# ohinder/OnePhase.jl

Measured on AMD Instinct MI355X. Metric: KKT factor+solve/sec (fp64) at n+m~1e5, nnz~2e6, higher is better.
Workload: dtype f64

## Files before the change

onephase.jl_amd/csrc/solve.hip:

```cpp
#include "numeric.h"
#include "solve_sparse.h"

#include <algorithm>
#include <cstdio>
#include <cstdlib>

namespace okkt {

#define OKKT_HIP_TRY(expr)                                                         \
  do {                                                                             \
    hipError_t e__ = (expr);                                                       \
    if (e__ != hipSuccess)                                                         \
      return std::string(#expr) + ": " + hipGetErrorString(e__);                   \
  } while (0)

typedef double d4_t __attribute__((ext_vector_type(4)));
typedef double d2_t __attribute__((ext_vector_type(2)));

constexpr int kSB = kSolveBlock;
#ifndef OKKT_SOLVE_SPLITS
#define OKKT_SOLVE_SPLITS 8
#endif
constexpr int kCS = OKKT_SOLVE_SPLITS;
static_assert(kSB / kCS >= 128 && (kCS & (kCS - 1)) == 0, "the block-product kernels need column splits of at least 128 columns (64 gave wrong results: found in round 3)");
// ... 482 lines not shown
  }
  const int kq = min(CW, pend - q0);
  const double* X = P.xinv + P.xinv_pos[s] + off + (size_t)q0 * ld;
  const int ic = min(i, kb - 1);
  const int64_t gcb = P.bigcol_base[s];
  if (ver && b > 0) flow_wait(ver, (c0 + q0) >> 5, ((c0 + q0 + kq - 1) >> 5) - ((c0 + q0) >> 5) + 1, vwant, nullptr, 0ull, P.counters + 5);
  for (int c = tid; c < CW; c += 256) {
    double w[R];
#pragma unroll
    for (int r = 0; r < R; ++r) w[r] = 0.0;
    if (c < kq) {
      if (b == 0) fwd_gather<R>(P, gcb, col0, k, q0 + c, w);
      else {
#pragma unroll
        for (int r = 0; r < R; ++r) w[r] = ver ? ld_agent(&P.xwork[(size_t)r * P.xw_stride + col0 + c0 + q0 + c]) : P.xwork[(size_t)r * P.xw_stride + col0 + c0 + q0 + c];
      }
    }
#pragma unroll
    for (int r = 0; r < R; ++r) wj[r][c] = w[r];
  }
  __syncthreads();
  double a[R];
#pragma unroll
  for (int r = 0; r < R; ++r) a[r] = 0.0;
  for (int p0 = wv * (CW / 4); p0 < min(kq, (wv + 1) * (CW / 4)); p0 += 32) {
    double v[32];
#pragma unroll
    for (int q = 0; q < 32; ++q) v[q] = X[(size_t)min(p0 + q, kq - 1) * ld + ic];
#pragma unroll
    for (int q = 0; q < 32; ++q) {
      const double vv = p0 + q < kq ? v[q] : 0.0;
#pragma unroll
      for (int r = 0; r < R; ++r) a[r] += vv * wj[r][min(p0 + q, CW - 1)];
    }
  }
#pragma unroll
  for (int r = 0; r < R; ++r) part[wv][r][lane] = a[r];
  __syncthreads();
  if (wv == 0 && i < kb)
#pragma unroll
    for (int r = 0; r < R; ++r) {
      const double v = (part[0][r][lane] + part[1][r][lane]) + (part[2][r][lane] + part[3][r][lane]);
      if (AG) st_agent(&yp[(size_t)r * kCS * kSB + i], v); else yp[(size_t)r * kCS * kSB + i] = v;
    }
  return true;
}
template <int R>
__global__ __launch_bounds__(256) void k_fwd_y(DevPlan P, const int* __restrict__ list, int b) {
  if (P.solve_mid) { const int s = list[blockIdx.y]; if (P.sn_col0[s + 1] - P.sn_col0[s] <= P.solve_mid) return; }
  (void)fwd_y_body<R, false>(P, list[blockIdx.y], b, (int)blockIdx.x, (int)blockIdx.z);
}

constexpr int kUpdRows = 64;
template <int R, int ROWS = kUpdRows>
__device__ __forceinline__ void fwd_upd_body(const DevPlan& P, int s, int b, int bx, double* sm, const unsigned long long* counter, unsigned long long epoch,
                                             unsigned long long* ver = nullptr, unsigned long long vbase = 0, int rb_abs = -1, int first = -1, long long yexp = -1) {
  constexpr int GW = ROWS / 2, NG = 256 / GW;
  double* yj = sm;
  double* part = sm + (size_t)R * kSB;
  const int tid = threadIdx.x, l32 = tid % GW, hw = tid / GW;
  const int col0 = P.sn_col0[s];
  const int k = P.sn_col0[s + 1] - col0;
  const int f = (int)(P.row_ptr[s + 1] - P.row_ptr[s]);
  int c0, kb, ld; int64_t off;
  xblock(k, b, c0, kb, ld, off);
  if (kb <= 0) return;
  const int rbeg = c0 + kb;
  const int rb = rb_abs >= 0 ? rb_abs : rbeg + bx * ROWS;
  const bool is_first = first >= 0 ? first != 0 : bx == 0;
  if (!is_first && rb >= f) return;
  const int vt0 = rb >> 5, vnt = rb < f ? min(ROWS / 32, (f - rb + 31) >> 5) : 0;
  if (ver) flow_wait(ver, vt0, b > 0 ? vnt : 0, vbase + (unsigned long long)b, counter, (epoch << 20) + (unsigned long long)yexp, P.counters + 5);
  else if (counter) front_wait64(counter, epoch, ((kb + 63) / 64) * kCS, P.counters + 5);
  const double* yp = P.ypart + P.ypart_pos[s] + (ver ? (size_t)b * kMaxRhs * kCS * kSB : 0);
  for (int p = tid; p < kSB; p += 256) {
    const int pc = min(p, kb - 1);
#pragma unroll
    for (int r = 0; r < R; ++r) {
      const double y = counter ? sum_splits_agent(yp + (size_t)r * kCS * kSB + pc) : sum_splits(yp + (size_t)r * kCS * kSB + pc);
      yj[r * kSB + p] = p < kb ? y : 0.0;
      if (is_first && p < kb) P.zwork[(size_t)r * P.xw_stride + col0 + c0 + p] = y / P.dvals[col0 + c0 + p];
    }
  }
  __syncthreads();
  if (rb >= f) return;
  const int r0 = rb + 2 * l32;
  const bool pair_ok = f >= 2;
  const int pr = pair_ok ? max(min(r0, f - 2), 0) : 0;
  const double* Lp = P.arena + P.front_pos[s] + (size_t)c0 * f + pr;
  double a0[R], a1[R];
#pragma unroll
  for (int r = 0; r < R; ++r) { a0[r] = 0.0; a1[r] = 0.0; }
  for (int p0 = hw; p0 < kb; p0 += 16 * NG) {
    d2_t v[16];
#pragma unroll
    for (int u = 0; u < 16; ++u) {
      const int p = min(p0 + NG * u, kb - 1);
      if (pair_ok) __builtin_memcpy(&v[u], Lp + (size_t)p * f, 16);
      else { v[u][0] = Lp[(size_t)p * f]; v[u][1] = 0.0; }
    }
#pragma unroll
    for (int u = 0; u < 16; ++u) {
      const int p = p0 + NG * u;
      if (p < kb) {
#pragma unroll
        for (int r = 0; r < R; ++r) { const double y = yj[r * kSB + p]; a0[r] += v[u][0] * y; a1[r] += v[u][1] * y; }
      }
    }
  }
#pragma unroll
  for (int r = 0; r < R; ++r) {
    part[((size_t)hw * R + r) * ROWS + 2 * l32] = a0[r];
    part[((size_t)hw * R + r) * ROWS + 2 * l32 + 1] = a1[r];
  }
  __syncthreads();
  if (tid < ROWS) {
    const int ln = tid >> 1, e = tid & 1;
    const int r0l = rb + 2 * ln;
    const int prl = pair_ok ? max(min(r0l, f - 2), 0) : 0;
    const int sh = r0l - prl;
    const int rowv = pair_ok ? prl + e : prl;
    const bool valid = pair_ok ? (sh == 0 || (sh == 1 && e == 1)) : (e == 0 && r0l < f);
    if (valid && rowv >= rbeg && rowv < f) {
      const int64_t gcb = P.bigcol_base[s];
      double w[R];
      if (b == 0) fwd_gather<R>(P, gcb, col0, k, rowv, w);
      else {
#pragma unroll
        for (int r = 0; r < R; ++r) w[r] = ver ? ld_agent(fwd_slot<R>(P, s, col0, k, rowv, r)) : *fwd_slot<R>(P, s, col0, k, rowv, r);
      }
#pragma unroll
      for (int r = 0; r < R; ++r) {
        double sum = 0.0;
#pragma unroll
        for (int h = 0; h < NG; ++h) sum += part[((size_t)h * R + r) * ROWS + tid];
        if (ver) st_agent(fwd_slot<R>(P, s, col0, k, rowv, r), w[r] - sum); else *fwd_slot<R>(P, s, col0, k, rowv, r) = w[r] - sum;
      }
    }
  }
  if (ver) flow_publish(ver, vt0, vnt, vbase + (unsigned long long)b + 1ull);
}

template <int R, int ROWS = kUpdRows>
__global__ __launch_bounds__(256) void k_fwd_upd(DevPlan P, const int* __restrict__ list, int b) {
  extern __shared__ __attribute__((aligned(16))) double sm[];
  fwd_upd_body<R, ROWS>(P, list[blockIdx.y], b, (int)blockIdx.x, sm, nullptr, 0ull);
}
template <int R>
__global__ __launch_bounds__(256) void k_fwd_wide_fused(DevPlan P, const int* __restrict__ list, int b, int ny, unsigned long long* __restrict__ counters, unsigned long long epoch) {
  extern __shared__ __attribute__((aligned(16))) double sm[];
  const int s = list[blockIdx.y];
  const int x = (int)blockIdx.x;
  if (x < ny * kCS) {
    if (fwd_y_body<R, true>(P, s, b, x % ny, x / ny)) front_arrive64(counters + s, epoch);
  } else {
    fwd_upd_body<R>(P, s, b, x - ny * kCS, sm, counters + s, epoch);
  }
}

constexpr int kFlowBlocks = 96;
constexpr int kFlowNear = 32;
struct SweepFlow {
  int nblk;
  int base[kFlowBlocks + 1];
  short nprod[kFlowBlocks];
};
template <int R>
__global__ __launch_bounds__(256) void k_fwd_wide_flow(DevPlan P, const int* __restrict__ list, SweepFlow T, unsigned long long* __restrict__ counters, unsigned long long epoch) {
  extern __shared__ __attribute__((aligned(16))) double sm[];
  const int s = list[blockIdx.x];
  const int t = (int)blockIdx.y;
  int b = 0;
  while (b + 1 < T.nblk && t >= T.base[b + 1]) ++b;
  const int idx = t - T.base[b];
  const int k = P.sn_col0[s + 1] - P.sn_col0[s];
  int c0, kb, ld; int64_t off;
  xblock(k, b, c0, kb, ld, off);
  if (kb <= 0) return;
  unsigned long long* ver = P.sver + P.sver_pos[s];
  const unsigned long long vbase = epoch << 12;
  const int nprod = T.nprod[b];
  const int f = (int)(P.row_ptr[s + 1] - P.row_ptr[s]);
  unsigned long long* ycnt = ver + ((f + 31) >> 5) + 2 + b;
  if (idx < nprod) {
    const int ny = nprod / kCS;
    if (fwd_y_body<R, true>(P, s, b, idx % ny, idx / ny, ver, vbase + (unsigned long long)b)) front_arrive64(ycnt, epoch);
    return;
  }
  const int j = idx - nprod;
  const int t0 = (c0 + kb) >> 5;
  const long long yexp = (long long)((kb + 63) / 64) * kCS;
  if (j < kFlowNear) fwd_upd_body<R, 32>(P, s, b, j, sm, ycnt, epoch, ver, vbase, 32 * (t0 + j), j == 0, yexp);
  else fwd_upd_body<R, 64>(P, s, b, j, sm, ycnt, epoch, ver, vbase, 32 * (t0 + kFlowNear) + 64 * (j - kFlowNear), 0, yexp);
}

template <int R, bool SC1>
__device__ __forceinline__ void bwd_pre_body(const DevPlan& P, int s, int xblk) {
  const int lane = threadIdx.x & 63, wv = threadIdx.x >> 6;
  const int col0 = P.sn_col0[s];
  const int k = P.sn_col0[s + 1] - col0;
  const int f = (int)(P.row_ptr[s + 1] - P.row_ptr[s]);
  const int c = xblk * 4 + wv;
  if (c >= k || f == k) return;
  const int* rows = P.rows + P.row_ptr[s];
  const double* col = P.arena + P.front_pos[s] + (size_t)c * f;
  double acc[R];
#pragma unroll
  for (int q = 0; q < R; ++q) acc[q] = 0.0;
  int r = k + lane;
  for (; r + 7 * 64 < f; r += 8 * 64) {
    int ri[8];
    double lv[8];
#pragma unroll
    for (int u = 0; u < 8; ++u) { ri[u] = rows[r + 64 * u]; lv[u] = col[r + 64 * u]; }
#pragma unroll
    for (int q = 0; q < R; ++q) {
      double xv[8];
#pragma unroll
      for (int u = 0; u < 8; ++u) xv[u] = P.xwork[(size_t)q * P.xw_stride + ri[u]];
#pragma unroll
      for (int u = 0; u < 8; ++u) acc[q] += lv[u] * xv[u];
    }
  }
  for (; r < f; r += 64) {
    const double l = col[r];
    const int g = rows[r];
#pragma unroll
    for (int q = 0; q < R; ++q) acc[q] += l * P.xwork[(size_t)q * P.xw_stride + g];
  }
#pragma unroll
  for (int q = 0; q < R; ++q) {
    double a = acc[q];
    for (int o = 32; o > 0; o >>= 1) a += __shfl_down(a, o, 64);
    if (lane == 0) {
      double* zp = &P.zwork[(size_t)q * P.xw_stride + col0 + c];
      if (SC1) st_agent(zp, *zp - a); else *zp -= a;
    }
  }
}
template <int R>
__global__ __launch_bounds__(256) void k_bwd_pre(DevPlan P, const int* __restrict__ list) {
  bwd_pre_body<R, false>(P, list[blockIdx.y], (int)blockIdx.x);
}

template <int R>
__device__ __forceinline__ void bwd_thin_body(const DevPlan& P, int s, int NB, int* counter, double (*tk)[128]) {
  const int tid = threadIdx.x;
  const int col0 = P.sn_col0[s];
  const int k = P.sn_col0[s + 1] - col0;
  const double* X = P.invl + P.invl_pos[s];
  const int c = tid >> 1, h = tid & 1;
  const double* xcol = X + (size_t)min(c, NB - 1) * NB;
  double v[64];
#pragma unroll
  for (int q = 0; q < 64; ++q) v[q] = xcol[min(h * 64 + q, NB - 1)];
  if (counter) {
    const int f = (int)(P.row_ptr[s + 1] - P.row_ptr[s]);
    const int expected = f > k ? (k + 3) / 4 : 0;
    front_wait(counter, expected, P.counters + 5);
    if (tid == 0) __hip_atomic_store(counter, 0, __ATOMIC_RELAXED, __HIP_MEMORY_SCOPE_AGENT);
  }
  if (tid < 128)
#pragma unroll
    for (int r = 0; r < R; ++r) {
      const double* zp = &P.zwork[(size_t)r * P.xw_stride + col0 + min(tid, max(k - 1, 0))];
      tk[r][tid] = tid < k ? (counter ? ld_agent(zp) : *zp) : 0.0;
    }
  __syncthreads();
#pragma unroll
  for (int r = 0; r < R; ++r) {
    double a = 0.0;
#pragma unroll
    for (int q = 0; q < 64; ++q) a += (h * 64 + q < NB) ? v[q] * tk[r][h * 64 + q] : 0.0;
    a += __shfl_xor(a, 1, 64);
    if (h == 0 && c < k) P.xwork[(size_t)r * P.xw_stride + col0 + c] = a;
  }
}
template <int R>
__global__ __launch_bounds__(256) void k_bwd_thin(DevPlan P, const int* __restrict__ list, int NB) {
  __shared__ double tk[R][128];
  bwd_thin_body<R>(P, list[blockIdx.x], NB, nullptr, tk);
}
template <int R>
__global__ __launch_bounds__(256) void k_bwd_thin_fused(DevPlan P, const int* __restrict__ list, int NB, int* __restrict__ counters) {
  __shared__ double tk[R][128];
  const int s = list[blockIdx.y];
  if (blockIdx.x + 1 < gridDim.x) {
    const int k = P.sn_col0[s + 1] - P.sn_col0[s];
    const int f = (int)(P.row_ptr[s + 1] - P.row_ptr[s]);
    if ((int)blockIdx.x * 4 >= k || f == k) return;
    bwd_pre_body<R, true>(P, s, (int)blockIdx.x);
    front_signal_add(counters + s);
  } else {
    bwd_thin_body<R>(P, s, NB, counters + s, tk);
  }
}

// ... 2 lines not shown
  constexpr int RW = kSB / kCS;
  __shared__ double zj[R][RW];
  const int tid = threadIdx.x, lane = tid & 63, wv = tid >> 6;
  const int col0 = P.sn_col0[s];
  const int k = P.sn_col0[s + 1] - col0;
  int c0, kb, ld; int64_t off;
  xblock(k, b, c0, kb, ld, off);
  if (kb <= 0) return false;
  if (bx * 64 >= kb) return false;
  double* xp = P.ypart + P.ypart_pos[s] + (size_t)rq * kSB;
  const int i0 = bx * 64 + wv * 16;
  const int q0 = rq * RW;
  if (q0 >= kb || q0 + RW - 1 < bx * 64) {
    if (lane < 16 && i0 + lane < kb)
#pragma unroll
      for (int r = 0; r < R; ++r) { if (AG) st_agent(&xp[(size_t)r * kCS * kSB + i0 + lane], 0.0); else xp[(size_t)r * kCS * kSB + i0 + lane] = 0.0; }
    return true;
  }
  const int kq = min(RW, kb - q0);
  const double* X = P.xinv + P.xinv_pos[s] + off + q0;
  for (int p = tid; p < RW; p += 256)
#pragma unroll
    for (int r = 0; r < R; ++r) zj[r][p] = p < kq ? P.zwork[(size_t)r * P.xw_stride + col0 + c0 + q0 + p] : 0.0;
  __syncthreads();
#pragma unroll 1
  for (int g = 0; g < 16; g += 4) {
    double v[4][RW / 64];
#pragma unroll
    for (int q = 0; q < 4; ++q) {
      const double* xc = X + (size_t)min(i0 + g + q, kb - 1) * ld;
#pragma unroll
      for (int t = 0; t < RW / 64; ++t) v[q][t] = xc[min(lane + 64 * t, kq - 1)];
    }
#pragma unroll
    for (int q = 0; q < 4; ++q) {
#pragma unroll
      for (int r = 0; r < R; ++r) {
        double a = 0.0;
#pragma unroll
        for (int t = 0; t < RW / 64; ++t) a += (lane + 64 * t < kq) ? v[q][t] * zj[r][lane + 64 * t] : 0.0;
        for (int o = 32; o > 0; o >>= 1) a += __shfl_down(a, o, 64);
        if (lane == 0 && i0 + g + q < kb) { if (AG) st_agent(&xp[(size_t)r * kCS * kSB + i0 + g + q], a); else xp[(size_t)r * kCS * kSB + i0 + g + q] = a; }
      }
    }
  }
  return true;
}
template <int R>
__global__ __launch_bounds__(256) void k_bwd_x(DevPlan P, const int* __restrict__ list, int b) {
  if (P.solve_mid) { const int s = list[blockIdx.y]; if (P.sn_col0[s + 1] - P.sn_col0[s] <= P.solve_mid) return; }
  (void)bwd_x_body<R, false>(P, list[blockIdx.y], b, (int)blockIdx.x, (int)blockIdx.z);
}

template <int R, int COLS = 64>
__device__ __forceinline__ void bwd_upd_body(const DevPlan& P, int s, int b, int bx, double* sm, const unsigned long long* counter, unsigned long long epoch) {
  const int tid = threadIdx.x, lane = tid & 63, wv = tid >> 6;
  const int col0 = P.sn_col0[s];
  const int k = P.sn_col0[s + 1] - col0;
  const int f = (int)(P.row_ptr[s + 1] - P.row_ptr[s]);
  int c0, kb, ld; int64_t off;
  xblock(k, b, c0, kb, ld, off);
  if (kb <= 0) return;
  const int nupd = (c0 + COLS - 1) / COLS;
  if (bx > nupd) return;
  if (counter) front_wait64(counter, epoch, ((kb + 63) / 64) * kCS, P.counters + 5);
  const double* xp = P.ypart + P.ypart_pos[s];
  for (int p = tid; p < kSB; p += 256) {
    const int pc = min(p, kb - 1);
#pragma unroll
    for (int r = 0; r < R; ++r) {
      const double x = counter ? sum_splits_agent(xp + (size_t)r * kCS * kSB + pc) : sum_splits(xp + (size_t)r * kCS * kSB + pc);
      sm[r * kSB + p] = p < kb ? x : 0.0;
    }
  }
  __syncthreads();
  if (bx == nupd) {
    for (int p = tid; p < kb; p += 256)
#pragma unroll
      for (int r = 0; r < R; ++r) P.xwork[(size_t)r * P.xw_stride + col0 + c0 + p] = sm[r * kSB + p];
    return;
  }
  const double* Lrow = P.arena + P.front_pos[s] + c0;
#pragma unroll 1
  for (int g = 0; g < COLS / 4; g += 2) {
    const int cb = bx * COLS + wv * (COLS / 4) + g;
    if (cb >= c0) break;
    double acc[2][R];
#pragma unroll
    for (int q = 0; q < 2; ++q)
#pragma unroll
      for (int r = 0; r < R; ++r) acc[q][r] = 0.0;
    for (int t0 = 0; t0 < kb; t0 += 64 * 16) {
      double v[2][16];
#pragma unroll
      for (int q = 0; q < 2; ++q) {
        const double* col = Lrow + (size_t)min(cb + q, c0 - 1) * f;
#pragma unroll
        for (int t = 0; t < 16; ++t) v[q][t] = col[min(t0 + lane + 64 * t, kb - 1)];
      }
#pragma unroll
      for (int t = 0; t < 16; ++t) {
        const int p = t0 + lane + 64 * t;
        if (p < kb) {
#pragma unroll
          for (int r = 0; r < R; ++r) {
            const double x = sm[r * kSB + p];
            acc[0][r] += v[0][t] * x;
            acc[1][r] += v[1][t] * x;
          }
        }
      }
    }
#pragma unroll
    for (int q = 0; q < 2; ++q)
#pragma unroll
      for (int r = 0; r < R; ++r) {
        double a = acc[q][r];
        for (int o = 32; o > 0; o >>= 1) a += __shfl_down(a, o, 64);
        if (lane == 0 && cb + q < c0) P.zwork[(size_t)r * P.xw_stride + col0 + cb + q] -= a;
      }
  }
}
template <int R, int COLS = 64>
__global__ __launch_bounds__(256) void k_bwd_upd(DevPlan P, const int* __restrict__ list, int b) {
  extern __shared__ __attribute__((aligned(16))) double sm[];
  bwd_upd_body<R, COLS>(P, list[blockIdx.y], b, (int)blockIdx.x, sm, nullptr, 0ull);
}
template <int R>
__global__ __launch_bounds__(256) void k_bwd_wide_fused(DevPlan P, const int* __restrict__ list, int b, int nx, unsigned long long* __restrict__ counters, unsigned long long epoch) {
  extern __shared__ __attribute__((aligned(16))) double sm[];
  const int s = list[blockIdx.y];
  const int x = (int)blockIdx.x;
  if (x < nx * kCS) {
    if (bwd_x_body<R, true>(P, s, b, x % nx, x / nx)) front_arrive64(counters + s, epoch);
  } else {
    bwd_upd_body<R>(P, s, b, x - nx * kCS, sm, counters + s, epoch);
  }
}

constexpr int kMidThreads = 1024;
__device__ __forceinline__ void mid_load_x(const double* Xb, int o, int NB, double (&xr)[4]) {
  const int tid = threadIdx.x;
#pragma unroll
  for (int u = 0; u < 4; ++u) {
    const int idx = tid + kMidThreads * u, i = idx & 63, j = idx >> 6;
    xr[u] = Xb[(o + i) + (size_t)(o + j) * NB];
  }
}
__device__ __forceinline__ void mid_store_x(const double (&xr)[4], double* xb) {
  const int tid = threadIdx.x;
#pragma unroll
  for (int u = 0; u < 4; ++u) {
    const int idx = tid + kMidThreads * u, i = idx & 63, j = idx >> 6;
    xb[i + j * 65] = xr[u];
  }
}
template <int R>
__global__ __launch_bounds__(kMidThreads) void k_fwd_mid(DevPlan P, const int* __restrict__ list, int NB) {
  extern __shared__ __attribute__((aligned(16))) double sm[];
  __shared__ double xb[2][64 * 65], ys[R][64];
  double (*part)[R][64] = (double (*)[R][64])(sm + (size_t)R * kSB);
  const int s = list[blockIdx.x];
  const int tid = threadIdx.x;
  const int col0 = P.sn_col0[s];
  const int k = P.sn_col0[s + 1] - col0;
  const int f = (int)(P.row_ptr[s + 1] - P.row_ptr[s]);
  if (k > P.solve_mid) return;
  const double* F = P.arena + P.front_pos[s];
  const double* X = P.invl + P.invl_pos[s];
  const int q = tid & 3, pr = tid >> 2;
  auto load_panel = [&](int c0, int pbase, d2_t (&v)[16]) {
    const int nb = min(64, k - c0);
    const int p = pbase + 2 * pr;
    if (c0 < k && p < k) {
      const bool two = p + 1 < k;
      const double* Lr = F + (size_t)(c0 + 16 * q) * f + (two ? p : p - 1);
#pragma unroll
      for (int u = 0; u < 16; ++u) __builtin_memcpy(&v[u], Lr + (size_t)min(u, max(nb - 1 - 16 * q, 0)) * f, 16);
    }
// ... 316 lines not shown
        ssched.push_back(s);
        L.wide_maxf = std::max(L.wide_maxf, N.sn_f[s]); L.wide_maxk = std::max(L.wide_maxk, N.sn_k[s]); L.wide_mink = std::min(L.wide_mink, N.sn_k[s]);
        if (xinv_pos[s] < 0) {
          const int64_t k = N.sn_k[s];
          const int64_t nfull = k / kSB, last = k - nfull * kSB, lastp = (last + 127) / 128 * 128;
          xinv_pos[s] = xtot;
          xtot += nfull * (int64_t)kSB * kSB + lastp * lastp;
          ypart_pos[s] = ytot;
          ytot += (int64_t)kMaxRhs * kCS * kSB * (N.solve_flow ? (k + kSB - 1) / kSB : 1);
          sver_pos[s] = vtot;
          vtot += (N.sn_f[s] + 31) / 32 + 2 + (k + kSB - 1) / kSB;
        }
      }
    }
  };
  build(N.levels, N.slevels);
  build(N.levels_top, N.slevels_top);
  std::string e;
  if (!(e = up(N, ssched, &d.ssched)).empty()) return e;
  N.ssched_host = ssched;
  if (!(e = up(N, xinv_pos, &d.xinv_pos)).empty()) return e;
  if (!(e = up(N, ypart_pos, &d.ypart_pos)).empty()) return e;
  if (!(e = up(N, ythin_pos, &d.ythin_pos)).empty()) return e;
  if (!(e = dz(N, (size_t)ttot, &d.ythin)).empty()) return e;
  if (!(e = dz(N, (size_t)xtot, &d.xinv)).empty()) return e;
  if (!(e = dz(N, (size_t)xtot, &d.xtmp)).empty()) return e;
  if (!(e = dz(N, (size_t)ytot, &d.ypart)).empty()) return e;
  if (!(e = up(N, sver_pos, &d.sver_pos)).empty()) return e;
  {
    double* rawv = nullptr;
    if (!(e = dz(N, (size_t)vtot + 1, &rawv)).empty()) return e;
    d.sver = (unsigned long long*)rawv;
  }
  {
    double* raw = nullptr;
    if (!(e = dz(N, (size_t)ns + 64, &raw)).empty()) return e;
    N.solve_flags = (int*)raw;
    N.solve_counters = (int*)raw + ns + 16;
    N.solve_epoch = 0;
    double* raw64 = nullptr;
    if (!(e = dz(N, (size_t)ns + 8, &raw64)).empty()) return e;
    N.solve_counters64 = (unsigned long long*)raw64;
    N.solve_epoch64 = 0;
  }
  for (const void* fn : {(const void*)k_fwd_wide_fused<1>, (const void*)k_fwd_wide_fused<2>, (const void*)k_fwd_wide_fused<4>, (const void*)k_bwd_wide_fused<1>,
                         (const void*)k_bwd_wide_fused<2>, (const void*)k_bwd_wide_fused<4>})
    OKKT_HIP_TRY(hipFuncSetAttribute(fn, hipFuncAttributeMaxDynamicSharedMemorySize, 160 * 1024 - 4096 - 16 * 1024));
  for (const void* fn : {(const void*)k_fwd_mid<1>, (const void*)k_fwd_mid<2>, (const void*)k_fwd_mid<4>, (const void*)k_bwd_mid<1>, (const void*)k_bwd_mid<2>, (const void*)k_bwd_mid<4>})
    OKKT_HIP_TRY(hipFuncSetAttribute(fn, hipFuncAttributeMaxDynamicSharedMemorySize, 80 * 1024));
  for (const void* fn : {(const void*)k_fwd_upd<1>, (const void*)k_fwd_upd<2>, (const void*)k_fwd_upd<4>, (const void*)k_bwd_upd<1>,
                         (const void*)k_bwd_upd<2>, (const void*)k_bwd_upd<4>, (const void*)k_fwd_upd<1, 32>, (const void*)k_fwd_upd<2, 32>, (const void*)k_fwd_upd<4, 32>, (const void*)k_bwd_upd<1, 16>, (const void*)k_bwd_upd<2, 16>, (const void*)k_bwd_upd<4, 16>, (const void*)k_fs_small<256, 1>, (const void*)k_fs_small<256, 2>,
                         (const void*)k_fs_small<256, 4>, (const void*)k_bs_small<256, 1>, (const void*)k_bs_small<256, 2>, (const void*)k_bs_small<256, 4>})
    OKKT_HIP_TRY(hipFuncSetAttribute(fn, hipFuncAttributeMaxDynamicSharedMemorySize, 160 * 1024 - 4096));
  return "";
}

std::string solve_invert_enqueue(Numeric& N, hipStream_t st, const SolveLevel& L, int b_lo, int b_hi) {
  if (!L.wide_cnt) return "";
  DevPlan P = N.d;
  const int* list = P.ssched + L.wide_off;
  const int nblk = (L.wide_maxk + kSB - 1) / kSB;
  b_hi = std::min(b_hi, nblk);
  if (b_lo >= b_hi) return "";
  const int nbk = b_hi - b_lo;
  const int maxkb = std::min(kSB, L.wide_maxk - b_lo * kSB);
  const int ldmax = std::min(kSB, (maxkb + 127) / 128 * 128);
  hipLaunchKernelGGL(k_xinv_init, dim3(ldmax / N.nb, 1, (unsigned)(L.wide_cnt * nbk)), dim3(256), 0, st, P, list, b_lo, nbk, N.nb);
  for (int sz = N.nb; sz < ldmax; sz *= 2) {
    const int npair = (ldmax + 2 * sz - 1) / (2 * sz);
    const int tiles = ((sz + 63) / 64) * ((sz + 63) / 64);
    hipLaunchKernelGGL(k_xinv_gemm<0>, dim3(tiles, npair, (unsigned)(L.wide_cnt * nbk)), dim3(256), 0, st, P, list, b_lo, nbk, sz);
    hipLaunchKernelGGL(k_xinv_gemm<1>, dim3(tiles, npair, (unsigned)(L.wide_cnt * nbk)), dim3(256), 0, st, P, list, b_lo, nbk, sz);
  }
  OKKT_HIP_TRY(hipGetLastError());
  return "";
}

struct SweepView {
  const std::vector<LevelSchedule>& levels;
  const std::vector<SolveLevel>& sl;
  const int* sched;
  const int* ssched;
  bool own, waits;
};

template <int R>
static std::string fwd_enqueue_r(Numeric& N, const SweepView& V, hipStream_t st, int l_lo, int l_hi) {
  DevPlan P = N.d;
  const std::vector<LevelSchedule>& levels = V.levels;
  const std::vector<SolveLevel>& sl = V.sl;
  const bool flow = V.own && V.waits && N.flow_levels >= 2 && N.flow_flags && l_lo == 0 && l_hi >= N.flow_levels;
  for (size_t l = (size_t)l_lo; l < std::min((size_t)l_hi, levels.size()); ++l) {
    const LevelSchedule& L = levels[l];
    if (flow && l == 0) {
      const size_t lds = (size_t)R * N.flow_maxf * sizeof(double);
      int* flags = N.flow_flags + (size_t)N.d.nsuper;
      const int ep = ++N.flow_epoch;
      static const int drop = getenv("OKKT_DEBUG_DROP_HANDOFF") ? atoi(getenv("OKKT_DEBUG_DROP_HANDOFF")) : 0;
      const int wep = ep + ((drop & 2) ? (1 << 20) : 0);
      if (N.flow_maxf <= 32) hipLaunchKernelGGL((k_fs_small<64, R, true>), dim3(N.flow_cnt), dim3(64), lds, st, P, P.sched + N.flow_off, N.flow_maxf, flags, ep, wep);
      else hipLaunchKernelGGL((k_fs_small<256, R, true>), dim3(N.flow_cnt), dim3(256), lds, st, P, P.sched + N.flow_off, N.flow_maxf, flags, ep, wep);
      l = (size_t)N.flow_levels - 1;
      continue;
    }
    for (int c = 0; c < 3; ++c) {
      const Segment& g = L.seg[c];
      if (!g.cnt) continue;
      const size_t lds = (size_t)R * g.maxf * sizeof(double);
      if (c == 0) hipLaunchKernelGGL((k_fs_small<64, R>), dim3(g.cnt), dim3(64), lds, st, P, V.sched + g.off, g.maxf, (int*)nullptr, 0, 0);
      else hipLaunchKernelGGL((k_fs_small<256, R>), dim3(g.cnt), dim3(256), lds, st, P, V.sched + g.off, g.maxf, (int*)nullptr, 0, 0);
    }
    if (V.own && (size_t)l < N.inv_level_pending.size() && N.inv_level_pending[l]) {
      OKKT_HIP_TRY(hipStreamWaitEvent(st, N.inv_level_events[l], 0));
      N.inv_level_pending[l] = 0;
    }
    const SolveLevel& S = sl[l];
    if (S.thin_cnt && V.waits && N.solve_fuse && N.solve_flags) {
      hipLaunchKernelGGL(k_fwd_thin_fused<R>, dim3((S.thin_maxr + 127) / 128 + 1, S.thin_cnt), dim3(256), 0, st, P, V.ssched + S.thin_off, N.nb, N.solve_flags, N.solve_epoch);
    } else if (S.thin_cnt) {
      hipLaunchKernelGGL(k_fwd_thin_y<R>, dim3(S.thin_cnt), dim3(256), 0, st, P, V.ssched + S.thin_off, N.nb);
      if (S.thin_maxr > 0) hipLaunchKernelGGL(k_fwd_thin_upd<R>, dim3((S.thin_maxr + 127) / 128, S.thin_cnt), dim3(256), 0, st, P, V.ssched + S.thin_off);
    }
    if (S.wide_cnt) {
      const int* list = V.ssched + S.wide_off;
      const int nblk = (S.wide_maxk + kSB - 1) / kSB;
      const size_t lds = ((size_t)R * kSB + (size_t)8 * R * kUpdRows) * sizeof(double);
      bool flow_done = false;
      if (V.waits && N.solve_flow && N.solve_counters64 && P.sver && nblk <= kFlowBlocks) {
        SweepFlow T;
        T.nblk = nblk;
        int64_t tot = 0;
        for (int b = 0; b < nblk; ++b) {
          const int kbmax = std::min(kSB, S.wide_maxk - b * kSB);
          const int rem = std::max(S.wide_maxf - b * kSB, 0);
          T.base[b] = (int)tot;
          T.nprod[b] = (short)(((kbmax + 63) / 64) * kCS);
          tot += T.nprod[b] + kFlowNear + std::max(0, (rem + 32 - 32 * kFlowNear + 63) / 64);
        }
        T.base[nblk] = (int)tot;
        if (tot <= 65535) {
          hipLaunchKernelGGL(k_fwd_wide_flow<R>, dim3(S.wide_cnt, (unsigned)tot), dim3(256), lds, st, P, list, T, N.solve_counters64, ++N.solve_epoch64);
          flow_done = true;
        }
      }
      for (int b = 0; b < nblk && !flow_done; ++b) {
        const int kbmax = std::min(kSB, S.wide_maxk - b * kSB);
        const int rem = std::max(S.wide_maxf - b * kSB, 0);
        const int ny = (kbmax + 63) / 64, nupd = std::max(1, (rem + kUpdRows - 1) / kUpdRows);
        if (V.waits && N.solve_fuse && N.solve_counters64 && ny * kCS * S.wide_cnt <= N.solve_fuse_wide_max) {
          hipLaunchKernelGGL(k_fwd_wide_fused<R>, dim3(ny * kCS + nupd, S.wide_cnt), dim3(256), lds, st, P, list, b, ny, N.solve_counters64, ++N.solve_epoch64);
        } else {
          if (P.solve_mid && b == 0 && S.wide_mink <= P.solve_mid) hipLaunchKernelGGL(k_fwd_mid<R>, dim3(S.wide_cnt), dim3(kMidThreads), (size_t)R * (kSB + 16 * 64) * sizeof(double), st, P, list, N.nb);
          if (!P.solve_mid || S.wide_maxk > P.solve_mid) hipLaunchKernelGGL(k_fwd_y<R>, dim3(ny, S.wide_cnt, kCS), dim3(256), 0, st, P, list, b);
          if (N.solve_split_small && nupd * S.wide_cnt < N.solve_split_small) hipLaunchKernelGGL((k_fwd_upd<R, 32>), dim3(std::max(1, (rem + 31) / 32), S.wide_cnt), dim3(256), lds, st, P, list, b);
          else hipLaunchKernelGGL(k_fwd_upd<R>, dim3(nupd, S.wide_cnt), dim3(256), lds, st, P, list, b);
        }
      }
    }
  }
  OKKT_HIP_TRY(hipGetLastError());
  return "";
}

template <int R>
static std::string bwd_enqueue_r(Numeric& N, const SweepView& V, hipStream_t st, int l_lo, int l_hi) {
  DevPlan P = N.d;
  const std::vector<LevelSchedule>& levels = V.levels;
  const std::vector<SolveLevel>& sl = V.sl;
  const bool flow = V.own && V.waits && N.flow_levels >= 2 && N.flow_flags && l_lo == 0 && l_hi >= N.flow_levels;
  for (int l = std::min(l_hi, (int)levels.size()) - 1; l >= l_lo; --l) {
    const LevelSchedule& L = levels[l];
    if (flow && l == N.flow_levels - 1) {
      const size_t lds = (size_t)R * N.flow_maxf * sizeof(double);
      int* flags = N.flow_flags + (size_t)2 * N.d.nsuper;
      const int ep = ++N.flow_epoch;
      if (N.flow_maxf <= 32) hipLaunchKernelGGL((k_bs_small<64, R, true>), dim3(N.flow_cnt), dim3(64), lds, st, P, P.sched + N.flow_off, N.flow_maxf, flags, ep);
      else hipLaunchKernelGGL((k_bs_small<256, R, true>), dim3(N.flow_cnt), dim3(256), lds, st, P, P.sched + N.flow_off, N.flow_maxf, flags, ep);
      break;
    }
    const SolveLevel& S = sl[l];
    if (S.wide_cnt) {
      const int* list = V.ssched + S.wide_off;
      if (S.wide_maxf > 0) hipLaunchKernelGGL(k_bwd_pre<R>, dim3((S.wide_maxk + 3) / 4, S.wide_cnt), dim3(256), 0, st, P, list);
      const int nblk = (S.wide_maxk + kSB - 1) / kSB;
      const size_t lds = (size_t)R * kSB * sizeof(double);
      for (int b = nblk - 1; b >= 0; --b) {
        const int kbmax = std::min(kSB, S.wide_maxk - b * kSB);
        const int nx = (kbmax + 63) / 64, nupd = (b * kSB + 63) / 64 + 1;
        if (V.waits && N.solve_fuse && N.solve_counters64 && nx * kCS * S.wide_cnt <= N.solve_fuse_wide_max) {
          hipLaunchKernelGGL(k_bwd_wide_fused<R>, dim3(nx * kCS + nupd, S.wide_cnt), dim3(256), lds, st, P, list, b, nx, N.solve_counters64, ++N.solve_epoch64);
        } else {
          if (P.solve_mid && b == 0 && S.wide_mink <= P.solve_mid) hipLaunchKernelGGL(k_bwd_mid<R>, dim3(S.wide_cnt), dim3(kMidThreads), (size_t)R * (kSB + 16 * 64) * sizeof(double), st, P, list, N.nb);
          if (!P.solve_mid || S.wide_maxk > P.solve_mid) hipLaunchKernelGGL(k_bwd_x<R>, dim3(nx, S.wide_cnt, kCS), dim3(256), 0, st, P, list, b);
          if (P.solve_mid && S.wide_maxk <= P.solve_mid) continue;
          if (N.solve_split_small && nupd * S.wide_cnt < N.solve_split_small) hipLaunchKernelGGL((k_bwd_upd<R, 16>), dim3((b * kSB + 15) / 16 + 1, S.wide_cnt), dim3(256), lds, st, P, list, b);
          else hipLaunchKernelGGL(k_bwd_upd<R>, dim3(nupd, S.wide_cnt), dim3(256), lds, st, P, list, b);
        }
      }
    }
    if (S.thin_cnt && V.waits && N.solve_fuse && N.solve_counters) {
      hipLaunchKernelGGL(k_bwd_thin_fused<R>, dim3((S.thin_maxk + 3) / 4 + 1, S.thin_cnt), dim3(256), 0, st, P, V.ssched + S.thin_off, N.nb, N.solve_counters);
    } else if (S.thin_cnt) {
      const int* list = V.ssched + S.thin_off;
      if (S.thin_maxr > 0) hipLaunchKernelGGL(k_bwd_pre<R>, dim3((S.thin_maxk + 3) / 4, S.thin_cnt), dim3(256), 0, st, P, list);
      hipLaunchKernelGGL(k_bwd_thin<R>, dim3(S.thin_cnt), dim3(256), 0, st, P, list, N.nb);
    }
    for (int c = 0; c < 3; ++c) {
      const Segment& g = L.seg[c];
      if (!g.cnt) continue;
      const size_t lds = (size_t)R * g.maxf * sizeof(double);
      if (c == 0) hipLaunchKernelGGL((k_bs_small<64, R>), dim3(g.cnt), dim3(64), lds, st, P, V.sched + g.off, g.maxf, (int*)nullptr, 0);
      else hipLaunchKernelGGL((k_bs_small<256, R>), dim3(g.cnt), dim3(256), lds, st, P, V.sched + g.off, g.maxf, (int*)nullptr, 0);
    }
  }
  OKKT_HIP_TRY(hipGetLastError());
  return "";
}


static std::string sweep(Numeric& N, bool fwd, const SweepView& V, hipStream_t st, int R, int l_lo = 0, int l_hi = 1 << 30) {
  if (fwd) return R == 1 ? fwd_enqueue_r<1>(N, V, st, l_lo, l_hi) : (R == 2 ? fwd_enqueue_r<2>(N, V, st, l_lo, l_hi) : fwd_enqueue_r<4>(N, V, st, l_lo, l_hi));
  return R == 1 ? bwd_enqueue_r<1>(N, V, st, l_lo, l_hi) : (R == 2 ? bwd_enqueue_r<2>(N, V, st, l_lo, l_hi) : bwd_enqueue_r<4>(N, V, st, l_lo, l_hi));
}

static std::string sweep_which(Numeric& N, bool fwd, int which, int R) {
  if (which != 0) return sweep(N, fwd, SweepView{N.levels_top, N.slevels_top, N.d.sched, N.d.ssched, false, true}, N.stream, R);
  return sweep(N, fwd, SweepView{N.levels, N.slevels, N.d.sched, N.d.ssched, true, true}, N.stream, R);
}

std::string solve_fwd_enqueue(Numeric& N, int which, int R) {
  if (which == 0 && N.inv_wait) { OKKT_HIP_TRY(hipStreamWaitEvent(N.stream, N.inv_event, 0)); N.inv_wait = false; }
  ++N.solve_epoch;
  return sweep_which(N, true, which, R);
}
std::string solve_bwd_enqueue(Numeric& N, int which, int R) {
  return sweep_which(N, false, which, R);
}

std::string solve_fwd_enqueue_lists(Numeric& N, const SweepLists& L, int R) {
  if (N.inv_wait) { OKKT_HIP_TRY(hipStreamWaitEvent(N.stream, N.inv_event, 0)); N.inv_wait = false; }
  ++N.solve_epoch;
  return sweep(N, true, SweepView{*L.levels, *L.slevels, L.sched, L.ssched, true, false}, N.stream, R);
}
std::string solve_bwd_enqueue_lists(Numeric& N, const SweepLists& L, int R) {
  return sweep(N, false, SweepView{*L.levels, *L.slevels, L.sched, L.ssched, true, false}, N.stream, R);
}

std::string schur_gather_enqueue(Numeric& N, double* d_r2, int nr, int R) {
  const int ns = N.sn_k[N.schur_sn], col0 = N.d.n - ns;
// ... 74 lines not shown
```

Measured before the change: 57.90.

## Software-pipeline panel loads in sparse triangular solve update kernels and tile backward pre-pass

Adds a PIPE variant of the forward and backward block-update kernels. It issues the first panel load before waiting on the y/x partial sums, then alternates two register buffers so the next column group loads while the current one is accumulated. It also adds a new backward pre-pass kernel that stages gathered x values through double-buffered shared memory in 512-row chunks, with one column per half-wave. All of these are on by default through environment toggles. The cost is more registers per thread, which may lower occupancy, and the extra prefetches read clamped, redundant data.

```diff
diff --git a/onephase.jl_amd/csrc/solve.hip b/onephase.jl_amd/csrc/solve.hip
--- a/onephase.jl_amd/csrc/solve.hip
+++ b/onephase.jl_amd/csrc/solve.hip
@@ -558,7 +558,7 @@
 }
 
 constexpr int kUpdRows = 64;
-template <int R, int ROWS = kUpdRows>
+template <int R, int ROWS = kUpdRows, bool PIPE = false>
 __device__ __forceinline__ void fwd_upd_body(const DevPlan& P, int s, int b, int bx, double* sm, const unsigned long long* counter, unsigned long long epoch,
                                              unsigned long long* ver = nullptr, unsigned long long vbase = 0, int rb_abs = -1, int first = -1, long long yexp = -1) {
   constexpr int GW = ROWS / 2, NG = 256 / GW;
@@ -576,20 +576,6 @@
   const bool is_first = first >= 0 ? first != 0 : bx == 0;
   if (!is_first && rb >= f) return;
   const int vt0 = rb >> 5, vnt = rb < f ? min(ROWS / 32, (f - rb + 31) >> 5) : 0;
-  if (ver) flow_wait(ver, vt0, b > 0 ? vnt : 0, vbase + (unsigned long long)b, counter, (epoch << 20) + (unsigned long long)yexp, P.counters + 5);
-  else if (counter) front_wait64(counter, epoch, ((kb + 63) / 64) * kCS, P.counters + 5);
-  const double* yp = P.ypart + P.ypart_pos[s] + (ver ? (size_t)b * kMaxRhs * kCS * kSB : 0);
-  for (int p = tid; p < kSB; p += 256) {
-    const int pc = min(p, kb - 1);
-#pragma unroll
-    for (int r = 0; r < R; ++r) {
-      const double y = counter ? sum_splits_agent(yp + (size_t)r * kCS * kSB + pc) : sum_splits(yp + (size_t)r * kCS * kSB + pc);
-      yj[r * kSB + p] = p < kb ? y : 0.0;
-      if (is_first && p < kb) P.zwork[(size_t)r * P.xw_stride + col0 + c0 + p] = y / P.dvals[col0 + c0 + p];
-    }
-  }
-  __syncthreads();
-  if (rb >= f) return;
   const int r0 = rb + 2 * l32;
   const bool pair_ok = f >= 2;
   const int pr = pair_ok ? max(min(r0, f - 2), 0) : 0;
@@ -597,14 +583,15 @@
   double a0[R], a1[R];
 #pragma unroll
   for (int r = 0; r < R; ++r) { a0[r] = 0.0; a1[r] = 0.0; }
-  for (int p0 = hw; p0 < kb; p0 += 16 * NG) {
-    d2_t v[16];
+  auto load_cols = [&](int p0, d2_t (&v)[16]) {
 #pragma unroll
     for (int u = 0; u < 16; ++u) {
       const int p = min(p0 + NG * u, kb - 1);
-      if (pair_ok) __builtin_memcpy(&v[u], Lp + (size_t)p * f, 16);
+      if (PIPE || pair_ok) __builtin_memcpy(&v[u], Lp + (size_t)p * f, 16);
       else { v[u][0] = Lp[(size_t)p * f]; v[u][1] = 0.0; }
     }
+  };
+  auto fma_cols = [&](int p0, const d2_t (&v)[16]) {
 #pragma unroll
     for (int u = 0; u < 16; ++u) {
       const int p = p0 + NG * u;
@@ -612,6 +599,56 @@
 #pragma unroll
         for (int r = 0; r < R; ++r) { const double y = yj[r * kSB + p]; a0[r] += v[u][0] * y; a1[r] += v[u][1] * y; }
       }
+    }
+  };
+  d2_t va[16];
+  if (PIPE && rb < f) load_cols(hw, va);
+  if (ver) flow_wait(ver, vt0, b > 0 ? vnt : 0, vbase + (unsigned long long)b, counter, (epoch << 20) + (unsigned long long)yexp, P.counters + 5);
+  else if (counter) front_wait64(counter, epoch, ((kb + 63) / 64) * kCS, P.counters + 5);
+  const double* yp = P.ypart + P.ypart_pos[s] + (ver ? (size_t)b * kMaxRhs * kCS * kSB : 0);
+  if (PIPE) {
+    double y[kSB / 256][R], dv[kSB / 256];
+#pragma unroll
+    for (int i = 0; i < kSB / 256; ++i) {
+      const int pc = min(tid + 256 * i, kb - 1);
+#pragma unroll
+      for (int r = 0; r < R; ++r) y[i][r] = sum_splits(yp + (size_t)r * kCS * kSB + pc);
+      dv[i] = P.dvals[col0 + c0 + pc];
+    }
+#pragma unroll
+    for (int i = 0; i < kSB / 256; ++i) {
+      const int p = tid + 256 * i;
+#pragma unroll
+      for (int r = 0; r < R; ++r) {
+        yj[r * kSB + p] = p < kb ? y[i][r] : 0.0;
+        if (is_first && p < kb) P.zwork[(size_t)r * P.xw_stride + col0 + c0 + p] = y[i][r] / dv[i];
+      }
+    }
+  } else {
+    for (int p = tid; p < kSB; p += 256) {
+      const int pc = min(p, kb - 1);
+#pragma unroll
+      for (int r = 0; r < R; ++r) {
+        const double y = counter ? sum_splits_agent(yp + (size_t)r * kCS * kSB + pc) : sum_splits(yp + (size_t)r * kCS * kSB + pc);
+        yj[r * kSB + p] = p < kb ? y : 0.0;
+        if (is_first && p < kb) P.zwork[(size_t)r * P.xw_stride + col0 + c0 + p] = y / P.dvals[col0 + c0 + p];
+      }
+    }
+  }
+  __syncthreads();
+  if (rb >= f) return;
+  if (PIPE) {
+    d2_t vb[16];
+    for (int p0 = hw; p0 - hw < kb; p0 += 32 * NG) {
+      load_cols(p0 + 16 * NG, vb);
+      fma_cols(p0, va);
+      load_cols(p0 + 32 * NG, va);
+      fma_cols(p0 + 16 * NG, vb);
+    }
+  } else {
+    for (int p0 = hw; p0 < kb; p0 += 16 * NG) {
+      load_cols(p0, va);
+      fma_cols(p0, va);
     }
   }
 #pragma unroll
@@ -647,10 +684,10 @@
   if (ver) flow_publish(ver, vt0, vnt, vbase + (unsigned long long)b + 1ull);
 }
 
-template <int R, int ROWS = kUpdRows>
+template <int R, int ROWS = kUpdRows, bool PIPE = false>
 __global__ __launch_bounds__(256) void k_fwd_upd(DevPlan P, const int* __restrict__ list, int b) {
   extern __shared__ __attribute__((aligned(16))) double sm[];
-  fwd_upd_body<R, ROWS>(P, list[blockIdx.y], b, (int)blockIdx.x, sm, nullptr, 0ull);
+  fwd_upd_body<R, ROWS, PIPE>(P, list[blockIdx.y], b, (int)blockIdx.x, sm, nullptr, 0ull);
 }
 template <int R>
 __global__ __launch_bounds__(256) void k_fwd_wide_fused(DevPlan P, const int* __restrict__ list, int b, int ny, unsigned long long* __restrict__ counters, unsigned long long epoch) {
@@ -749,6 +786,98 @@
   bwd_pre_body<R, false>(P, list[blockIdx.y], (int)blockIdx.x);
 }
 
+constexpr int kPreTile = 8, kPreChunk = 512;
+template <int R>
+__device__ __forceinline__ void bwd_pre_tile_body(const DevPlan& P, int s, int xblk, double (*xs)[R][kPreChunk]) {
+  constexpr int NL = kPreChunk / 64, NS = kPreChunk / 256;
+  static_assert(kPreTile == 8, "one column per half-wave of a 256-thread workgroup");
+  const int tid = threadIdx.x, hl = tid & 31;
+  const int col0 = P.sn_col0[s];
+  const int k = P.sn_col0[s + 1] - col0;
+  const int f = (int)(P.row_ptr[s + 1] - P.row_ptr[s]);
+  const int cfirst = xblk * kPreTile;
+  if (cfirst >= k || f == k) return;
+  const int nr = f - k, nch = (nr + kPreChunk - 1) / kPreChunk;
+  const int* rows = P.rows + P.row_ptr[s] + k;
+  const int cw = cfirst + (tid >> 5);
+  const double* col = P.arena + P.front_pos[s] + (size_t)min(cw, k - 1) * f;
+  auto load_idx = [&](int ch, int (&ri)[NS]) {
+#pragma unroll
+    for (int j = 0; j < NS; ++j) ri[j] = rows[min(ch * kPreChunk + tid + 256 * j, nr - 1)];
+  };
+  auto load_x = [&](const int (&ri)[NS], double (&xg)[NS][R]) {
+#pragma unroll
+    for (int j = 0; j < NS; ++j)
+#pragma unroll
+      for (int q = 0; q < R; ++q) xg[j][q] = P.xwork[(size_t)q * P.xw_stride + ri[j]];
+  };
+  auto store_x = [&](int ch, const double (&xg)[NS][R]) {
+#pragma unroll
+    for (int j = 0; j < NS; ++j)
+#pragma unroll
+      for (int q = 0; q < R; ++q) xs[ch & 1][q][tid + 256 * j] = ch * kPreChunk + tid + 256 * j < nr ? xg[j][q] : 0.0;
+  };
+  auto load_panel = [&](int ch, d2_t (&v)[NL]) {
+#pragma unroll
+    for (int u = 0; u < NL; ++u) {
+      const int rseg = k + ch * kPreChunk + 64 * u;
+      __builtin_memcpy(&v[u], col + min(rseg + 2 * hl, f - 2), 16);
+    }
+  };
+  double acc0[R], acc1[R];
+#pragma unroll
+  for (int q = 0; q < R; ++q) { acc0[q] = 0.0; acc1[q] = 0.0; }
+  auto consume = [&](int ch, const d2_t (&v)[NL]) {
+#pragma unroll
+    for (int u = 0; u < NL; ++u) {
+      const int r0 = k + ch * kPreChunk + 64 * u + 2 * hl;
+      const int sh = r0 - min(r0, f - 2);
+      const double l0 = sh == 0 ? v[u][0] : (sh == 1 ? v[u][1] : 0.0);
+      const double l1 = sh == 0 ? v[u][1] : 0.0;
+#pragma unroll
+      for (int q = 0; q < R; ++q) {
+        d2_t x;
+        __builtin_memcpy(&x, &xs[ch & 1][q][64 * u + 2 * hl], 16);
+        acc0[q] += l0 * x[0];
+        acc1[q] += l1 * x[1];
+      }
+    }
+  };
+  int ri[NS];
+  double xg[NS][R];
+  d2_t va[NL], vb[NL];
+  load_idx(0, ri);
+  load_panel(0, va);
+  load_x(ri, xg);
+  load_idx(1, ri);
+  store_x(0, xg);
+  __syncthreads();
+  auto step = [&](int n, d2_t (&cur)[NL], d2_t (&nxt)[NL]) {
+    load_x(ri, xg);
+    load_idx(n + 2, ri);
+    load_panel(n + 1, nxt);
+    consume(n, cur);
+    store_x(n + 1, xg);
+    __syncthreads();
+  };
+  for (int n = 0; n < nch; n += 2) {
+    step(n, va, vb);
+    step(n + 1, vb, va);
+  }
+#pragma unroll
+  for (int q = 0; q < R; ++q) {
+    double a0 = acc0[q], a1 = acc1[q];
+    for (int o = 16; o > 0; o >>= 1) { a0 += __shfl_down(a0, o, 64); a1 += __shfl_down(a1, o, 64); }
+    const double a = a0 + a1;
+    if (hl == 0 && cw < k) P.zwork[(size_t)q * P.xw_stride + col0 + cw] -= a;
+  }
+}
+template <int R>
+__global__ __launch_bounds__(256) void k_bwd_pre_tile(DevPlan P, const int* __restrict__ list) {
+  __shared__ __attribute__((aligned(16))) double xs[2][R][kPreChunk];
+  bwd_pre_tile_body<R>(P, list[blockIdx.y], (int)blockIdx.x, xs);
+}
+
 template <int R>
 __device__ __forceinline__ void bwd_thin_body(const DevPlan& P, int s, int NB, int* counter, double (*tk)[128]) {
   const int tid = threadIdx.x;
@@ -857,7 +986,7 @@
   (void)bwd_x_body<R, false>(P, list[blockIdx.y], b, (int)blockIdx.x, (int)blockIdx.z);
 }
 
-template <int R, int COLS = 64>
+template <int R, int COLS = 64, bool PIPE = false>
 __device__ __forceinline__ void bwd_upd_body(const DevPlan& P, int s, int b, int bx, double* sm, const unsigned long long* counter, unsigned long long epoch) {
   const int tid = threadIdx.x, lane = tid & 63, wv = tid >> 6;
   const int col0 = P.sn_col0[s];
@@ -868,6 +997,54 @@
   if (kb <= 0) return;
   const int nupd = (c0 + COLS - 1) / COLS;
   if (bx > nupd) return;
+  const double* Lrow = P.arena + P.front_pos[s] + c0;
+  const int cw = bx * COLS + wv * (COLS / 4);
+  const int nt = (kb + 64 * 16 - 1) / (64 * 16);
+  const int nit = bx < nupd ? (COLS / 8) * nt : 0;
+  auto load_item = [&](int i, double (&v)[2][16]) {
+    const int cb = cw + 2 * (i / nt), t0 = (i % nt) * 64 * 16;
+    if (i >= nit || cb >= c0) return;
+#pragma unroll
+    for (int q = 0; q < 2; ++q) {
+      const double* col = Lrow + (size_t)min(cb + q, c0 - 1) * f;
+#pragma unroll
+      for (int t = 0; t < 16; ++t) v[q][t] = col[min(t0 + lane + 64 * t, kb - 1)];
+    }
+  };
+  double pacc[2][R];
+  auto use_item = [&](int i, const double (&v)[2][16]) {
+    const int cb = cw + 2 * (i / nt), t0 = (i % nt) * 64 * 16;
+    if (i >= nit || cb >= c0) return;
+    if (t0 == 0) {
+#pragma unroll
+      for (int q = 0; q < 2; ++q)
+#pragma unroll
+        for (int r = 0; r < R; ++r) pacc[q][r] = 0.0;
+    }
+#pragma unroll
+    for (int t = 0; t < 16; ++t) {
+      const int p = t0 + lane + 64 * t;
+      if (p < kb) {
+#pragma unroll
+        for (int r = 0; r < R; ++r) {
+          const double x = sm[r * kSB + p];
+          pacc[0][r] += v[0][t] * x;
+          pacc[1][r] += v[1][t] * x;
+        }
+      }
+    }
+    if (t0 + 64 * 16 < kb) return;
+#pragma unroll
+    for (int q = 0; q < 2; ++q)
+#pragma unroll
+      for (int r = 0; r < R; ++r) {
+        double a = pacc[q][r];
+        for (int o = 32; o > 0; o >>= 1) a += __shfl_down(a, o, 64);
+        if (lane == 0 && cb + q < c0) P.zwork[(size_t)r * P.xw_stride + col0 + cb + q] -= a;
+      }
+  };
+  double pva[2][16];
+  if (PIPE) load_item(0, pva);
   if (counter) front_wait64(counter, epoch, ((kb + 63) / 64) * kCS, P.counters + 5);
   const double* xp = P.ypart + P.ypart_pos[s];
   for (int p = tid; p < kSB; p += 256) {
@@ -885,51 +1062,27 @@
       for (int r = 0; r < R; ++r) P.xwork[(size_t)r * P.xw_stride + col0 + c0 + p] = sm[r * kSB + p];
     return;
   }
-  const double* Lrow = P.arena + P.front_pos[s] + c0;
+  if (PIPE) {
+    double pvb[2][16];
 #pragma unroll 1
-  for (int g = 0; g < COLS / 4; g += 2) {
-    const int cb = bx * COLS + wv * (COLS / 4) + g;
-    if (cb >= c0) break;
-    double acc[2][R];
-#pragma unroll
-    for (int q = 0; q < 2; ++q)
-#pragma unroll
-      for (int r = 0; r < R; ++r) acc[q][r] = 0.0;
-    for (int t0 = 0; t0 < kb; t0 += 64 * 16) {
-      double v[2][16];
-#pragma unroll
-      for (int q = 0; q < 2; ++q) {
-        const double* col = Lrow + (size_t)min(cb + q, c0 - 1) * f;
-#pragma unroll
-        for (int t = 0; t < 16; ++t) v[q][t] = col[min(t0 + lane + 64 * t, kb - 1)];
-      }
-#pragma unroll
-      for (int t = 0; t < 16; ++t) {
-        const int p = t0 + lane + 64 * t;
-        if (p < kb) {
-#pragma unroll
-          for (int r = 0; r < R; ++r) {
-            const double x = sm[r * kSB + p];
-            acc[0][r] += v[0][t] * x;
-            acc[1][r] += v[1][t] * x;
-          }
-        }
-      }
-    }
-#pragma unroll
-    for (int q = 0; q < 2; ++q)
-#pragma unroll
-      for (int r = 0; r < R; ++r) {
-        double a = acc[q][r];
-        for (int o = 32; o > 0; o >>= 1) a += __shfl_down(a, o, 64);
-        if (lane == 0 && cb + q < c0) P.zwork[(size_t)r * P.xw_stride + col0 + cb + q] -= a;
-      }
-  }
-}
-template <int R, int COLS = 64>
+    for (int i = 0; i < nit; i += 2) {
+      load_item(i + 1, pvb);
+      use_item(i, pva);
+      load_item(i + 2, pva);
+      use_item(i + 1, pvb);
+    }
+  } else {
+#pragma unroll 1
+    for (int i = 0; i < nit; ++i) {
+      load_item(i, pva);
+      use_item(i, pva);
+    }
+  }
+}
+template <int R, int COLS = 64, bool PIPE = false>
 __global__ __launch_bounds__(256) void k_bwd_upd(DevPlan P, const int* __restrict__ list, int b) {
   extern __shared__ __attribute__((aligned(16))) double sm[];
-  bwd_upd_body<R, COLS>(P, list[blockIdx.y], b, (int)blockIdx.x, sm, nullptr, 0ull);
+  bwd_upd_body<R, COLS, PIPE>(P, list[blockIdx.y], b, (int)blockIdx.x, sm, nullptr, 0ull);
 }
 template <int R>
 __global__ __launch_bounds__(256) void k_bwd_wide_fused(DevPlan P, const int* __restrict__ list, int b, int nx, unsigned long long* __restrict__ counters, unsigned long long epoch) {
@@ -1352,6 +1505,10 @@
                          (const void*)k_bwd_upd<2>, (const void*)k_bwd_upd<4>, (const void*)k_fwd_upd<1, 32>, (const void*)k_fwd_upd<2, 32>, (const void*)k_fwd_upd<4, 32>, (const void*)k_bwd_upd<1, 16>, (const void*)k_bwd_upd<2, 16>, (const void*)k_bwd_upd<4, 16>, (const void*)k_fs_small<256, 1>, (const void*)k_fs_small<256, 2>,
                          (const void*)k_fs_small<256, 4>, (const void*)k_bs_small<256, 1>, (const void*)k_bs_small<256, 2>, (const void*)k_bs_small<256, 4>})
     OKKT_HIP_TRY(hipFuncSetAttribute(fn, hipFuncAttributeMaxDynamicSharedMemorySize, 160 * 1024 - 4096));
+  for (const void* fn : {(const void*)k_fwd_upd<1, kUpdRows, true>, (const void*)k_fwd_upd<2, kUpdRows, true>, (const void*)k_fwd_upd<4, kUpdRows, true>, (const void*)k_fwd_upd<1, 32, true>,
+                         (const void*)k_fwd_upd<2, 32, true>, (const void*)k_fwd_upd<4, 32, true>, (const void*)k_bwd_upd<1, 64, true>, (const void*)k_bwd_upd<2, 64, true>,
+                         (const void*)k_bwd_upd<4, 64, true>, (const void*)k_bwd_upd<1, 16, true>, (const void*)k_bwd_upd<2, 16, true>, (const void*)k_bwd_upd<4, 16, true>})
+    OKKT_HIP_TRY(hipFuncSetAttribute(fn, hipFuncAttributeMaxDynamicSharedMemorySize, 160 * 1024 - 4096));
   return "";
 }
 
@@ -1383,6 +1540,11 @@
   const int* ssched;
   bool own, waits;
 };
+
+static bool upd_pipe() {
+  static const int on = getenv("OKKT_SOLVE_UPD_PIPE") ? atoi(getenv("OKKT_SOLVE_UPD_PIPE")) : 1;
+  return on != 0;
+}
 
 template <int R>
 static std::string fwd_enqueue_r(Numeric& N, const SweepView& V, hipStream_t st, int l_lo, int l_hi) {
@@ -1452,8 +1614,12 @@
         } else {
           if (P.solve_mid && b == 0 && S.wide_mink <= P.solve_mid) hipLaunchKernelGGL(k_fwd_mid<R>, dim3(S.wide_cnt), dim3(kMidThreads), (size_t)R * (kSB + 16 * 64) * sizeof(double), st, P, list, N.nb);
           if (!P.solve_mid || S.wide_maxk > P.solve_mid) hipLaunchKernelGGL(k_fwd_y<R>, dim3(ny, S.wide_cnt, kCS), dim3(256), 0, st, P, list, b);
-          if (N.solve_split_small && nupd * S.wide_cnt < N.solve_split_small) hipLaunchKernelGGL((k_fwd_upd<R, 32>), dim3(std::max(1, (rem + 31) / 32), S.wide_cnt), dim3(256), lds, st, P, list, b);
-          else hipLaunchKernelGGL(k_fwd_upd<R>, dim3(nupd, S.wide_cnt), dim3(256), lds, st, P, list, b);
+          const bool rows32 = N.solve_split_small && nupd * S.wide_cnt < N.solve_split_small;
+          const dim3 ugrid(rows32 ? std::max(1, (rem + 31) / 32) : nupd, S.wide_cnt);
+          if (rows32 && upd_pipe()) hipLaunchKernelGGL((k_fwd_upd<R, 32, true>), ugrid, dim3(256), lds, st, P, list, b);
+          else if (rows32) hipLaunchKernelGGL((k_fwd_upd<R, 32>), ugrid, dim3(256), lds, st, P, list, b);
+          else if (upd_pipe()) hipLaunchKernelGGL((k_fwd_upd<R, kUpdRows, true>), ugrid, dim3(256), lds, st, P, list, b);
+          else hipLaunchKernelGGL(k_fwd_upd<R>, ugrid, dim3(256), lds, st, P, list, b);
         }
       }
     }
@@ -1481,7 +1647,9 @@
     const SolveLevel& S = sl[l];
     if (S.wide_cnt) {
       const int* list = V.ssched + S.wide_off;
-      if (S.wide_maxf > 0) hipLaunchKernelGGL(k_bwd_pre<R>, dim3((S.wide_maxk + 3) / 4, S.wide_cnt), dim3(256), 0, st, P, list);
+      static const int pre_tile = getenv("OKKT_SOLVE_PRE_TILE") ? atoi(getenv("OKKT_SOLVE_PRE_TILE")) : 1;
+      if (S.wide_maxf > 0 && pre_tile) hipLaunchKernelGGL(k_bwd_pre_tile<R>, dim3((S.wide_maxk + kPreTile - 1) / kPreTile, S.wide_cnt), dim3(256), 0, st, P, list);
+      else if (S.wide_maxf > 0) hipLaunchKernelGGL(k_bwd_pre<R>, dim3((S.wide_maxk + 3) / 4, S.wide_cnt), dim3(256), 0, st, P, list);
       const int nblk = (S.wide_maxk + kSB - 1) / kSB;
       const size_t lds = (size_t)R * kSB * sizeof(double);
       for (int b = nblk - 1; b >= 0; --b) {
@@ -1493,8 +1661,12 @@
           if (P.solve_mid && b == 0 && S.wide_mink <= P.solve_mid) hipLaunchKernelGGL(k_bwd_mid<R>, dim3(S.wide_cnt), dim3(kMidThreads), (size_t)R * (kSB + 16 * 64) * sizeof(double), st, P, list, N.nb);
           if (!P.solve_mid || S.wide_maxk > P.solve_mid) hipLaunchKernelGGL(k_bwd_x<R>, dim3(nx, S.wide_cnt, kCS), dim3(256), 0, st, P, list, b);
           if (P.solve_mid && S.wide_maxk <= P.solve_mid) continue;
-          if (N.solve_split_small && nupd * S.wide_cnt < N.solve_split_small) hipLaunchKernelGGL((k_bwd_upd<R, 16>), dim3((b * kSB + 15) / 16 + 1, S.wide_cnt), dim3(256), lds, st, P, list, b);
-          else hipLaunchKernelGGL(k_bwd_upd<R>, dim3(nupd, S.wide_cnt), dim3(256), lds, st, P, list, b);
+          const bool cols16 = N.solve_split_small && nupd * S.wide_cnt < N.solve_split_small;
+          const dim3 ugrid(cols16 ? (b * kSB + 15) / 16 + 1 : nupd, S.wide_cnt);
+          if (cols16 && upd_pipe()) hipLaunchKernelGGL((k_bwd_upd<R, 16, true>), ugrid, dim3(256), lds, st, P, list, b);
+          else if (cols16) hipLaunchKernelGGL((k_bwd_upd<R, 16>), ugrid, dim3(256), lds, st, P, list, b);
+          else if (upd_pipe()) hipLaunchKernelGGL((k_bwd_upd<R, 64, true>), ugrid, dim3(256), lds, st, P, list, b);
+          else hipLaunchKernelGGL(k_bwd_upd<R>, ugrid, dim3(256), lds, st, P, list, b);
         }
       }
     }
```

Measured after the change: 58.19, median of 6. Within noise of the previous version (+0.5%).
